# creare-com/pydem

Hardware: AMD Instinct MI355X
Metric: Mcells/s (slope+aspect+UCA+TWI end-to-end) per tile; % HBM roofline (higher is better)
Workload: dtype f64

## Files before the change

### pydem_amd/csrc/pits.hip

```cpp
#include "internal.h"
#include <hipcub/hipcub.hpp>
#include <math.h>
#include <stdlib.h>
#include <algorithm>
#include <vector>

namespace {

__device__ __forceinline__ double np_pairwise_leaf(const double *a, int n)
{
    if (n < 8) {
        double res = 0.;
        for (int i = 0; i < n; i++) res += a[i];
        return res;
    }
    double r0 = a[0], r1 = a[1], r2 = a[2], r3 = a[3], r4 = a[4], r5 = a[5], r6 = a[6], r7 = a[7];
    int i;
    for (i = 8; i < n - (n % 8); i += 8) {
        r0 += a[i]; r1 += a[i + 1]; r2 += a[i + 2]; r3 += a[i + 3];
        r4 += a[i + 4]; r5 += a[i + 5]; r6 += a[i + 6]; r7 += a[i + 7];
    }
    double res = ((r0 + r1) + (r2 + r3)) + ((r4 + r5) + (r6 + r7));
    for (; i < n; i++) res += a[i];
    return res;
// ... 1167 lines not shown
}

__global__ void k_pit_gather(const uint64_t *__restrict__ keys, const int32_t *__restrict__ idx, const double *__restrict__ w,
                             int32_t ne, int swap, int32_t *a, int32_t *b, double *wo, int32_t *dup, int kb)
{
    for (int32_t e = blockIdx.x * blockDim.x + threadIdx.x; e < ne; e += gridDim.x * blockDim.x) {
        const uint64_t k = keys[e];
        if (dup && e > 0 && keys[e - 1] == k) atomicAdd(dup, 1);
        const int32_t hi = (int32_t)(k >> kb), lo = (int32_t)(k & ((1ull << kb) - 1ull));
        a[e] = swap ? lo : hi;
        b[e] = swap ? hi : lo;
        wo[e] = w[idx[e]];
    }
}

template <typename T>
int dev_realloc(pydem_tile *t, T **p, size_t count)
{
    if (*p) { plane_give(t->device, *p); *p = nullptr; }
    return tile_alloc(t, p, count);
}

}

int stage_pits(pydem_tile *t, const pydem_options *opt)
{
    const int n = (int)t->n, m = (int)t->m;
    if (opt->drain_pits_max_iter > 300) {
        pydem_set_error("drain_pits_max_iter > 300 is not supported by the device window (got %d)", opt->drain_pits_max_iter);
        return -2;
    }
    HIP_TRY(hipEventRecord(t->ev[4], t->stream));
    PYDEM_TRY(tile_alloc(t, &t->flat0, (size_t)t->NN));
    PYDEM_TRY(tile_alloc(t, &t->flatlist, (size_t)t->NN));
    PYDEM_TRY(tile_alloc(t, &t->labels, (size_t)t->NN));
    PYDEM_TRY(tile_alloc(t, &t->queue[0], (size_t)t->NN));
    int32_t *cnt = t->counters + 40;
    HIP_TRY(hipMemsetAsync(cnt, 0, 16 * sizeof(int32_t), t->stream));
    const int big = (int)(cdiv(t->NN, 256) < 8192 ? cdiv(t->NN, 256) : 8192);
    hipLaunchKernelGGL(k_pitmask, dim3(big), dim3(256), 0, t->stream, t->flats, t->elev, t->NN, t->flat0);
    hipLaunchKernelGGL(k_compact_mask, dim3((unsigned)(cdiv(t->NN, 4096) < 4096 ? cdiv(t->NN, 4096) : 4096)), dim3(256), 0,
                       t->stream, t->flat0, t->NN, t->flatlist, cnt);
    HIP_TRY(hipMemcpyAsync(t->h_counters, cnt, sizeof(int32_t), hipMemcpyDeviceToHost, t->stream));
    HIP_TRY(hipStreamSynchronize(t->stream));
    const int32_t npits = t->h_counters[0];
    t->tm.n_pit_edges = 0; t->tm.n_pits_undrained = 0;
    t->tm.n_pits = npits; t->tm.n_pits_row = 0; t->tm.n_pits_wave = 0; t->tm.n_pits_big = 0;
    t->pits.n_edges = 0;
    if (npits == 0) { t->tm.pits_ms = 0; return 0; }

    int64_t cap = (int64_t)npits * 2 + 16384 * 4 * OUT_CHUNK + 1024;
    for (int attempt = 0;; attempt++) {
        if (t->pits.raw_cap < cap) {
            PYDEM_TRY(dev_realloc(t, &t->pits.raw_src, (size_t)cap));
            PYDEM_TRY(dev_realloc(t, &t->pits.raw_dst, (size_t)cap));
            PYDEM_TRY(dev_realloc(t, &t->pits.raw_w, (size_t)cap));
            t->pits.raw_cap = cap;
        }
        HIP_TRY(hipMemsetAsync(cnt + 1, 0, 8 * sizeof(int32_t), t->stream));
        PitParams P;
        P.dbg = nullptr; P.prof = nullptr;
        const char *dbg_env = getenv("PYDEM_PITS_DEBUG");
        if (dbg_env && atoi(dbg_env) == 3) { HIP_TRY(hipMalloc(&P.prof, 128)); HIP_TRY(hipMemsetAsync(P.prof, 0, 128, t->stream)); }
        if (dbg_env && atoi(dbg_env) >= 2) HIP_TRY(hipMalloc(&P.dbg, (size_t)npits * 16));
        HIP_TRY(hipMemsetAsync(t->pits.raw_src, 0xFF, (size_t)t->pits.raw_cap * 4, t->stream));
        P.elev = t->elev; P.pitmask = t->flat0; P.dX = t->dX; P.dY = t->dY; P.mag = t->mag; P.flats = t->flats;
        P.n = n; P.m = m; P.max_iter = opt->drain_pits_max_iter; P.max_dist = opt->drain_pits_max_dist;
        P.min_border = opt->drain_pits_min_border; P.max_dist_XY = opt->drain_pits_max_dist_XY;
        P.elev_f32 = t->elev_f32 ? 1 : 0;
        P.out_src = t->pits.raw_src; P.out_dst = t->pits.raw_dst; P.out_w = t->pits.raw_w;
        P.out_count = cnt + 1; P.out_cap = (int32_t)(t->pits.raw_cap < INT32_MAX ? t->pits.raw_cap : INT32_MAX);
        P.overflow_list = t->labels; P.overflow_count = cnt + 3;
        P.lane_overflow = t->queue[0];
        {
            static int handover = -1;
            if (handover < 0) { const char *e = getenv("PYDEM_PITS_HANDOVER"); handover = e ? atoi(e) : 1; }
            P.lane_state = nullptr;
            if (handover && (int64_t)npits * 12 <= t->NN) { PYDEM_TRY(tile_alloc(t, &t->queue[1], (size_t)t->NN)); P.lane_state = (uint32_t *)t->queue[1]; }
        }
        HIP_TRY(hipMemsetAsync(cnt + 10, 0, sizeof(int32_t), t->stream));
        P.work_next = cnt + 10;
        const int gl_cap = 3072 * 128 / LN_T;
        const int gl = (int)(cdiv(npits, LN_T) < gl_cap ? cdiv(npits, LN_T) : gl_cap);
        hipLaunchKernelGGL(k_pits_lane, dim3(gl), dim3(LN_T), 0, t->stream, P, t->flatlist, cnt);
        HIP_TRY(hipMemcpyAsync(t->h_counters, cnt, 8 * sizeof(int32_t), hipMemcpyDeviceToHost, t->stream));
        HIP_TRY(hipStreamSynchronize(t->stream));
        const int32_t n_lane_over = t->h_counters[5];
        if (P.prof) {
            unsigned long long h[8];
            HIP_TRY(hipMemcpy(h, P.prof, 64, hipMemcpyDeviceToHost));
            fprintf(stderr, "pits/lane: %llu loop trips over all wavefronts, %.1f busy lanes per trip; cycles: refill %llu, growth %llu, drain selection %llu, output %llu\n",
                    h[4], h[4] ? (double)h[3] / (double)h[4] : 0.0, h[0], h[5], h[1], h[2]);
        }
        int32_t n_row_over = -1, n_wave_over = 0, n_over = 0;
        P.wave_index = nullptr; P.row_overflow = nullptr; P.row_overflow_count = nullptr; P.row_rec = nullptr; P.rw_target = PYDEM_RW_TARGET;
        const char *row_env = getenv("PYDEM_PITS_ROW");
        const int row_mode = row_env ? atoi(row_env) : 1;
        const bool use_row = row_mode == 2 || (row_mode == 1 && n_lane_over >= 4 * 256 * PYDEM_WV_OCC);
        if (use_row && n_lane_over > 0 && 8 * (int64_t)n_lane_over + 64 <= t->NN) {
            HIP_TRY(hipMemsetAsync(cnt + 9, 0, 4 * sizeof(int32_t), t->stream));
            P.row_overflow = t->labels; P.row_overflow_count = cnt + 12;
            P.row_rec = (int2 *)(t->labels + (((size_t)t->NN / 2) & ~(size_t)63));
            const char *tgt_env = getenv("PYDEM_RW_TARGET");
            P.rw_target = tgt_env && atoi(tgt_env) > 0 ? atoi(tgt_env) : PYDEM_RW_TARGET;
            constexpr int per = RW_NT / 16, gr_cap = 256 * (RW_OCC * 256 / RW_NT);
            const int gr = (int)(cdiv(n_lane_over, per) < gr_cap ? cdiv(n_lane_over, per) : gr_cap);
            hipLaunchKernelGGL((k_pits_row<RW_CAP, RW_OCC, RW_NT>), dim3(gr), dim3(RW_NT), 0, t->stream, P, t->queue[0], cnt + 5);
            hipLaunchKernelGGL(k_pits_row_finish, dim3((unsigned)(cdiv(n_lane_over, 256) < 2048 ? cdiv(n_lane_over, 256) : 2048)), dim3(256), 0,
                               t->stream, P, t->queue[0], cnt + 5, P.row_rec);
            if (P.prof) {
                unsigned long long h[16];
                HIP_TRY(hipMemcpy(h, P.prof, 128, hipMemcpyDeviceToHost));
                fprintf(stderr, "pits/row: %llu loop trips over all wavefronts, %.2f busy / %.2f growing rows per trip, %llu refills; cycles: refill %llu, rounds %llu, drain selection %llu, output %llu\n",
                        h[12], h[12] ? (double)h[13] / (double)h[12] : 0.0, h[12] ? (double)h[14] / (double)h[12] : 0.0, h[15], h[8], h[9], h[10], h[11]);
            }
            P.wave_index = t->labels;
            P.overflow_list = t->labels + (((size_t)n_lane_over + 63) & ~(size_t)63);
            HIP_TRY(hipMemsetAsync(cnt + 10, 0, sizeof(int32_t), t->stream));
            const int gw = (int)(cdiv(n_lane_over, 4) < 256 * 4 ? cdiv(n_lane_over, 4) : 256 * 4);
            hipLaunchKernelGGL((k_pits_wave<512, 4>), dim3(gw), dim3(256), 0, t->stream, P, t->queue[0], cnt + 12);
            const int32_t *big_in = P.overflow_list;
            P.overflow_list = t->queue[0]; P.overflow_count = cnt + 9;
            P.wave_index = nullptr;
            hipLaunchKernelGGL(k_pits_wave_big, dim3(256), dim3(64), 0, t->stream, P, big_in, cnt + 3);
            HIP_TRY(hipMemcpyAsync(t->h_counters, cnt, 16 * sizeof(int32_t), hipMemcpyDeviceToHost, t->stream));
            HIP_TRY(hipStreamSynchronize(t->stream));
            n_row_over = t->h_counters[12]; n_wave_over = t->h_counters[3]; n_over = t->h_counters[9];
        } else {
            if (n_lane_over > 0) {
                const int gw = (int)(cdiv(n_lane_over, 4) < 256 * PYDEM_WV_OCC ? cdiv(n_lane_over, 4) : 256 * PYDEM_WV_OCC);
                HIP_TRY(hipMemsetAsync(cnt + 10, 0, sizeof(int32_t), t->stream));
                hipLaunchKernelGGL((k_pits_wave<PYDEM_WV_CAP, PYDEM_WV_OCC>), dim3(gw), dim3(256), 0, t->stream, P, t->queue[0], cnt + 5);
                HIP_TRY(hipMemcpyAsync(t->h_counters, cnt, 8 * sizeof(int32_t), hipMemcpyDeviceToHost, t->stream));
                HIP_TRY(hipStreamSynchronize(t->stream));
            }
            n_wave_over = t->h_counters[3];
            if (n_wave_over > 0) {
                HIP_TRY(hipMemsetAsync(cnt + 9, 0, sizeof(int32_t), t->stream));
                P.overflow_list = t->queue[0]; P.overflow_count = cnt + 9;
                hipLaunchKernelGGL(k_pits_wave_big, dim3(n_wave_over < 4096 ? n_wave_over : 4096), dim3(64), 0, t->stream, P, t->labels, cnt + 3);
                HIP_TRY(hipMemcpyAsync(t->h_counters, cnt, 16 * sizeof(int32_t), hipMemcpyDeviceToHost, t->stream));
                HIP_TRY(hipStreamSynchronize(t->stream));
                n_over = t->h_counters[9];
            }
        }
        if (P.prof) { (void)hipFree(P.prof); P.prof = nullptr; }
        t->tm.n_pits_row = n_row_over >= 0 ? n_lane_over : 0;
        t->tm.n_pits_wave = n_row_over >= 0 ? n_row_over : n_lane_over;
        t->tm.n_pits_big = n_wave_over;
        if (dbg_env) fprintf(stderr, "pits: %d candidates, %d left the 16x16 lane window, %d left the 64x64 row pass (-1: not run), %d left the 128x128 wavefront pass, %d left the 256x256 / 2048-cell pass, %d edge slots, %d undrained\n", npits, n_lane_over, n_row_over, n_wave_over, n_over, t->h_counters[1], t->h_counters[2]);
        if (P.dbg) {
            const int nrec = t->h_counters[7];
            std::vector<int32_t> rec((size_t)nrec * 4);
            HIP_TRY(hipMemcpy(rec.data(), P.dbg, rec.size() * 4, hipMemcpyDeviceToHost));
            (void)hipFree(P.dbg); P.dbg = nullptr;
            std::vector<int> rounds, border; int reason[4] = {0, 0, 0, 0}; long long tot_rounds = 0;
            for (int i = 0; i < nrec; i++) {
                rounds.push_back(rec[4 * i]); border.push_back(rec[4 * i + 1]); reason[rec[4 * i + 2] & 3]++; tot_rounds += rec[4 * i];
            }
            {
                const int edges[7] = {16, 32, 64, 128, 200, 299, 1 << 30};
                long long cr[7] = {0}, cn[7] = {0}, cd[7] = {0}, cu[7] = {0}, co[7] = {0};
                for (int i = 0; i < nrec; i++) {
                    int b = 0; while (rec[4 * i] > edges[b]) b++;
                    cr[b] += rec[4 * i]; cn[b]++;
                    if (rec[4 * i + 2] & 3) co[b]++; else if (rec[4 * i + 3] >= 0) cd[b]++; else cu[b]++;
// ... 115 lines not shown
```

### pydem_amd/csrc/uca.hip

```cpp
#include "uca_graph.h"
#include <algorithm>
#include <vector>
#include <math.h>
#include <stdlib.h>
#include <string.h>

#define PI_D 3.141592653589793

namespace {

__global__ __launch_bounds__(256) void k_section_proportion(const double *__restrict__ dir,
                                                            const uint8_t *__restrict__ flats,
                                                            const double *__restrict__ sec_theta, int64_t NN, int n, int m,
                                                            const double *__restrict__ elev,
                                                            int8_t *__restrict__ section, double *__restrict__ prop,
                                                            uint32_t *__restrict__ cinfo)
{
    (void)NN;
    for (int i = blockIdx.y; i < n; i += gridDim.y)
    for (int j = blockIdx.x * blockDim.x + threadIdx.x; j < m; j += gridDim.x * blockDim.x) {
        const int64_t c = (int64_t)i * m + j;
        const double theta = sec_theta[i];
        const double d = dir[c];
        int sec0 = (int)(int8_t)(int)floor(d / PI_D * 2.0);
        const double quadrant = d - PI_D / 2.0 * (double)sec0;
        const int mod2 = sec0 & 1;
        int sec = sec0 * 2 + ((quadrant > theta) && mod2 == 0) + ((quadrant > (PI_D / 2 - theta)) && mod2 == 1);
        sec = (int)(int8_t)sec;
        const bool I1 = sec == 0 || sec == 1 || sec == 4 || sec == 5;
        const double cth = PI_D / 2 - theta;
        const double t1 = I1 ? theta : cth, t2 = I1 ? cth : theta;
        const bool lo = quadrant <= t1, hi = quadrant > t1;
        const double num = lo ? quadrant : quadrant - t1, den = lo ? t1 : t2;
        double p = (lo || hi) ? num / den : NAN;
        if (flats[c]) { sec = -1; p = NAN; }
        if (sec == 8) sec = 0;
        const int a = (sec & 1) ? -1 : 1;
        const double pf = (1 + a) / 2.0 - (double)a * p;
        prop[c] = pf;
        section[c] = (int8_t)sec;
        uint32_t gf = 0;
        if (sec >= 0 && sec <= 7) {
            const double z = elev[c];
            const int i1 = i + fe1r(sec), j1 = j + fe1c(sec), i2 = i + fe2r(sec), j2 = j + fe2c(sec);
            if (i1 >= 0 && i1 < n && j1 >= 0 && j1 < m && keep_edge(pf, elev[(int64_t)i1 * m + j1], z)) gf |= CI_OUT1;
            if (i2 >= 0 && i2 < n && j2 >= 0 && j2 < m && keep_edge(1 - pf, elev[(int64_t)i2 * m + j2], z)) gf |= CI_OUT2;
        }
        cinfo[c] = gf | ((uint32_t)(sec & 7) << CI_SEC_SHIFT);
    }
}

__global__ __launch_bounds__(256) void k_graph_inmask(const double *__restrict__ prop, const double *__restrict__ elev,
                                                      int n, int m, uint32_t *__restrict__ cinfo, uint8_t *__restrict__ todo0,
                                                      uint8_t *__restrict__ todo_work, double *__restrict__ corner_sums)
{
    for (int i = blockIdx.y; i < n; i += gridDim.y)
    for (int j = blockIdx.x * blockDim.x + threadIdx.x; j < m; j += gridDim.x * blockDim.x) {
        const int64_t c = (int64_t)i * m + j;
        const uint32_t cw = cinfo[c] & (CI_OUT1 | CI_OUT2 | (7u << CI_SEC_SHIFT));
        uint32_t im = 0;
#pragma unroll
        for (int d = 0; d < 8; d++) {
            const int ui = i + NB_DI[d], uj = j + NB_DJ[d];
            if (ui < 0 || ui >= n || uj < 0 || uj >= m) continue;
            const uint32_t wu = cinfo[(int64_t)ui * m + uj];
            const int su = (int)((wu >> CI_SEC_SHIFT) & 7u);
            const bool cardinal = (NB_DI[d] == 0) || (NB_DJ[d] == 0);
            if ((su == NB_S0[d] || su == NB_S1[d]) && (wu & (cardinal ? CI_OUT1 : CI_OUT2))) im |= 1u << d;
        }
        cinfo[c] = im | cw | ((im ? CI_LEVEL_INF : 0u) << CI_LEVEL_SHIFT);
        const bool top = i == 0, bot = i == n - 1, left = j == 0, right = j == m - 1;
        if (top || bot || left || right) {
            const double TOL = 1e-2;
            const double p = prop[c], z = elev[c];
            double outsum = 0.0;
            if (cw & CI_OUT1) outsum += p;
            if (cw & CI_OUT2) outsum += 1 - p;
            const int s = (cw & (CI_OUT1 | CI_OUT2)) ? ci_section(cw) : -1;
            bool td = false;
            const bool has_out = outsum > TOL;
            if (left) td = has_out && (s == 6 || s == 7 || s == 0 || s == 1);
            if (right) td = has_out && (s == 2 || s == 3 || s == 4 || s == 5);
            if (top) td = has_out && (s == 4 || s == 5 || s == 6 || s == 7);
            if (bot) td = has_out && (s == 0 || s == 1 || s == 2 || s == 3);
            if ((top || bot) && (left || right)) {
                double insum = 0.0;
                for (int d = 0; d < 8; d++)
                    if (im & (1u << d)) {
                        const int64_t u = (int64_t)(i + NB_DI[d]) * m + (j + NB_DJ[d]);
                        const bool cardinal = (NB_DI[d] == 0) || (NB_DJ[d] == 0);
                        insum += cardinal ? prop[u] : 1 - prop[u];
                    }
                const int q = (top ? 0 : 2) + (left ? 0 : 1);
                corner_sums[q * 3 + 0] = outsum;
                corner_sums[q * 3 + 1] = insum;
                corner_sums[q * 3 + 2] = td ? 1.0 : 0.0;
            }
            if (isnan(z)) td = false;
            todo0[c] = td;
            todo_work[c] = td;
        }
    }
}

__global__ void k_graph_add_pits(const int32_t *__restrict__ src, const int32_t *__restrict__ dst,
                                 const double *__restrict__ w, int64_t ne, int n, int m,
                                 uint32_t *cinfo, double *corner_sums)
{
    for (int64_t e = (int64_t)blockIdx.x * blockDim.x + threadIdx.x; e < ne; e += (int64_t)gridDim.x * blockDim.x) {
        const int32_t s = src[e], d = dst[e];
        atomicOr(&cinfo[s], CI_PIT_OUT);
        atomicOr(&cinfo[d], CI_PIT_IN | (CI_LEVEL_INF << CI_LEVEL_SHIFT));
        const int corners[4] = {0, m - 1, (n - 1) * m, (n - 1) * m + m - 1};
        for (int q = 0; q < 4; q++) {
            if (s == corners[q]) atomicAdd(&corner_sums[q * 3 + 0], w[e]);
            if (d == corners[q]) atomicAdd(&corner_sums[q * 3 + 1], w[e]);
        }
    }
}

__global__ void k_corner_todo(const double *__restrict__ corner_sums, const double *__restrict__ elev, int n, int m,
                              uint8_t *todo0, uint8_t *todo_work)
{
    const int q = threadIdx.x;
    if (q >= 4) return;
    const int64_t corners[4] = {0, m - 1, (int64_t)(n - 1) * m, (int64_t)(n - 1) * m + m - 1};
    const int64_t c = corners[q];
    bool td = corner_sums[q * 3 + 2] != 0.0;
    td = td || (corner_sums[q * 3 + 0] > 1e-2) || (corner_sums[q * 3 + 1] < 1e-2);
    if (isnan(elev[c])) td = false;
    todo0[c] = td;
    todo_work[c] = td;
}

constexpr int STAGE_CAP = 4096;
constexpr int STAGE_FLUSH = STAGE_CAP - 512;


struct Stage {
    QE buf[STAGE_CAP];
    int32_t cnt;
    int32_t base;
};

__device__ __forceinline__ void stage_push(Stage &S, bool pred, int32_t cell, uint32_t cw)
{
    const unsigned long long bal = __ballot(pred);
    if (bal == 0ull) return;
    const int lane = (int)__lane_id();
    const int leader = __ffsll((long long)bal) - 1;
    int32_t base = 0;
    if (lane == leader) base = atomicAdd(&S.cnt, (int32_t)__popcll(bal));
    base = __shfl(base, leader);
    if (pred) { QE q; q.c = cell; q.cw = cw; S.buf[base + __popcll(bal & ((1ull << lane) - 1ull))] = q; }
}

__device__ __forceinline__ void stage_flush(const SweepArgs &A, Stage &S, QE *__restrict__ qn, int32_t *cn, bool force)
{
    __syncthreads();
    const int32_t c = S.cnt;
    if (c > 0 && (force || c > STAGE_FLUSH)) {
        if (threadIdx.x == 0) S.base = atomicAdd(cn, c);
        __syncthreads();
        const int32_t b = S.base;
        if ((int64_t)b + c <= A.qcap) { for (int32_t k = threadIdx.x; k < c; k += blockDim.x) qn[b + k] = S.buf[k]; }
        else if (threadIdx.x == 0) atomicAdd(A.err, 1);
        __syncthreads();
        if (threadIdx.x == 0) S.cnt = 0;
    }
    __syncthreads();
}

__device__ __forceinline__ int2 pit_stash(const SweepArgs &A, int32_t c) { return reinterpret_cast<const int2 *>(A.area)[c]; }

__global__ void k_pit_stash(const int32_t *__restrict__ pin_dst, const int32_t *__restrict__ pit_src, int64_t ne, double *area)
{
    int32_t *slots = reinterpret_cast<int32_t *>(area);
    for (int64_t e = (int64_t)blockIdx.x * blockDim.x + threadIdx.x; e < ne; e += (int64_t)gridDim.x * blockDim.x) {
        if (e == 0 || pin_dst[e - 1] != pin_dst[e]) slots[2 * (int64_t)pin_dst[e]] = (int32_t)e;
        if (e == 0 || pit_src[e - 1] != pit_src[e]) slots[2 * (int64_t)pit_src[e] + 1] = (int32_t)e;
    }
}

__device__ __forceinline__ void load_upstream_words(const SweepArgs &A, int32_t t, int ti, int tj, uint32_t w[8])
// ... 1401 lines not shown
template <bool WT = false>
__global__ __launch_bounds__(256) void k_reseed_gather(SweepArgs A, const ReseedCell *__restrict__ U, int32_t nU, const double *__restrict__ elev,
                                                       ReseedHost *__restrict__ out)
{
    for (int32_t k = blockIdx.x * blockDim.x + threadIdx.x; k < nU; k += gridDim.x * blockDim.x) {
        ReseedHost h;
        h.c = U[k].c; h.cw = A.cinfo[h.c] & CI_STATIC_MASK; h.pin_first = U[k].pin_first; h.pout_first = U[k].pout_first;
        double a; bool td;
        gather_finished<WT>(A, h.c, h.cw, h.pin_first, a, td);
        h.area = a; h.td = td; h.pad = 0; h.elev = elev[h.c]; h.prop = (h.cw & (CI_OUT1 | CI_OUT2)) ? A.prop[h.c] : 0.0;
        out[k] = h;
    }
}
struct ReseedBack { int32_t c; int32_t flags; double area; };
__global__ __launch_bounds__(256) void k_reseed_scatter(SweepArgs A, const ReseedBack *__restrict__ B, int32_t nU, uint32_t pass)
{
    for (int32_t k = blockIdx.x * blockDim.x + threadIdx.x; k < nU; k += gridDim.x * blockDim.x) {
        const int32_t c = B[k].c;
        A.area[c] = B[k].area;
        if (B[k].flags & 2) A.todo_work[c] = 1;
        if (B[k].flags & 1) A.cinfo[c] = ci_with_level(A.cinfo[c], pass);
    }
}

__device__ __forceinline__ bool finalize_cell(double *__restrict__ uca, const double *__restrict__ elev, int64_t c, uint32_t f, uint32_t td,
                                              int apply_limit, double limit)
{
    if (f) uca[c] = NAN;
    bool dn = !td;
    if (td && isnan(elev[c])) dn = true;
    if (apply_limit && !f && uca[c] > limit) dn = true;
    return dn;
}

__global__ __launch_bounds__(256) void k_uca_finalize(double *__restrict__ uca, const uint8_t *__restrict__ flats,
                                                      const uint8_t *__restrict__ todo_work, const double *__restrict__ elev,
                                                      uint8_t *__restrict__ edge_done, int64_t NN, int apply_limit, double limit)
{
    const int64_t nvec = NN >> 4, stride = (int64_t)gridDim.x * blockDim.x, t0 = (int64_t)blockIdx.x * blockDim.x + threadIdx.x;
    for (int64_t v = t0; v < nvec; v += stride) {
        const uint4 f4 = reinterpret_cast<const uint4 *>(flats)[v], t4 = reinterpret_cast<const uint4 *>(todo_work)[v];
        const uint32_t fw[4] = {f4.x, f4.y, f4.z, f4.w}, tw[4] = {t4.x, t4.y, t4.z, t4.w};
        uint32_t dw[4];
#pragma unroll
        for (int q = 0; q < 4; q++) {
            uint32_t d = 0;
#pragma unroll
            for (int b = 0; b < 4; b++)
                d |= (finalize_cell(uca, elev, v * 16 + q * 4 + b, (fw[q] >> (8 * b)) & 0xFFu, (tw[q] >> (8 * b)) & 0xFFu, apply_limit, limit) ? 1u : 0u) << (8 * b);
            dw[q] = d;
        }
        reinterpret_cast<uint4 *>(edge_done)[v] = make_uint4(dw[0], dw[1], dw[2], dw[3]);
    }
    for (int64_t c = (nvec << 4) + t0; c < NN; c += stride)
        edge_done[c] = finalize_cell(uca, elev, c, flats[c], todo_work[c], apply_limit, limit);
}

__global__ __launch_bounds__(256) void k_twi(const double *__restrict__ uca, const double *__restrict__ mag,
                                             double *__restrict__ twi, int64_t NN, double min_slope, int lim_uca,
                                             double uca_cap, int lim_twi, double twi_cap)
{
    for (int64_t c = (int64_t)blockIdx.x * blockDim.x + threadIdx.x; c < NN; c += (int64_t)gridDim.x * blockDim.x) {
        double t = uca[c];
        if (lim_uca && t > uca_cap) t = uca_cap;
        t = log(t / (mag[c] + min_slope));
        if (lim_twi && t > twi_cap) t = twi_cap;
        twi[c] = t;
    }
}

}

int stage_section_graph(pydem_tile *t, const pydem_options *opt)
{
    const int n = (int)t->n, m = (int)t->m;
    t->graph_opt = *opt;
    t->edge_clean = false;
    t->einc_ready = false;
    PYDEM_TRY(tile_alloc(t, &t->todo_work, (size_t)t->NN));
    PYDEM_TRY(tile_alloc(t, &t->cinfo, (size_t)t->NN));
    const dim3 grid2((unsigned)(cdiv(m, 256) < 64 ? cdiv(m, 256) : 64), (unsigned)(n < 16384 ? n : 16384));
    t->tm.n_pit_edges = 0; t->tm.n_pits_undrained = 0; t->tm.pits_ms = 0;
    t->pits.n_edges = 0; t->pits.n_raw = 0;
    double *corner_sums = (double *)(t->counters + CS_WORK);
    HIP_TRY(hipEventRecord(t->ev_fork, t->stream));
    HIP_TRY(hipStreamWaitEvent(t->stream2, t->ev_fork, 0));
    HIP_TRY(hipMemcpyAsync(t->todo_work, t->flats, (size_t)t->NN, hipMemcpyDeviceToDevice, t->stream2));
    HIP_TRY(hipEventRecord(t->ev_snap, t->stream2));
    HIP_TRY(hipStreamWaitEvent(t->stream, t->ev_snap, 0));
    hipLaunchKernelGGL(k_section_proportion, grid2, dim3(256), 0, t->stream2, t->dir, (const uint8_t *)t->todo_work, t->sec_theta,
                       t->NN, n, m, t->elev, t->section, t->prop, t->cinfo);
    HIP_TRY(hipMemsetAsync(t->counters + CS_WORK, 0, CS_WORK_WORDS * sizeof(int32_t), t->stream2));
    HIP_TRY(hipMemsetAsync(t->edge_todo, 0, (size_t)t->NN, t->stream2));
    HIP_TRY(hipMemsetAsync(t->todo_work, 0, (size_t)t->NN, t->stream2));
    hipLaunchKernelGGL(k_graph_inmask, grid2, dim3(256), 0, t->stream2, t->prop, t->elev, n, m,
                       t->cinfo, t->edge_todo, t->todo_work, corner_sums);
    HIP_TRY(hipEventRecord(t->ev_join, t->stream2));
    static int graph_serial = -1;
    if (graph_serial < 0) { const char *e = getenv("PYDEM_GRAPH_SERIAL"); graph_serial = e ? atoi(e) : 0; }
    if (graph_serial) HIP_TRY(hipStreamWaitEvent(t->stream, t->ev_join, 0));
    HIP_TRY(hipEventRecord(t->ev[0], t->stream));
    if (opt->drain_pits) PYDEM_TRY(stage_pits(t, opt));
    HIP_TRY(hipEventRecord(t->ev[2], t->stream));
    HIP_TRY(hipStreamWaitEvent(t->stream, t->ev_join, 0));
    if (t->pits.n_edges > 0) {
        hipLaunchKernelGGL(k_graph_add_pits, dim3(grid_for(t->pits.n_edges, 1024)), dim3(256), 0, t->stream, t->pits.src,
                           t->pits.dst, t->pits.w, t->pits.n_edges, n, m, t->cinfo, corner_sums);
    }
    hipLaunchKernelGGL(k_corner_todo, dim3(1), dim3(64), 0, t->stream, corner_sums, t->elev, n, m, t->edge_todo, t->todo_work);
    HIP_TRY(hipEventRecord(t->ev[3], t->stream));
    HIP_TRY(hipGetLastError());
    HIP_TRY(hipEventSynchronize(t->ev[3]));
    float a = 0, b = 0;
    HIP_TRY(hipEventElapsedTime(&a, t->ev[0], t->ev[2]));
    HIP_TRY(hipEventElapsedTime(&b, t->ev[2], t->ev[3]));
    (void)a;
    t->tm.graph_ms = b;
    return 0;
}


static int64_t reseed_replay_host(std::vector<ReseedHost> &H, std::vector<uint8_t> &done, int n, int m, int maxcount, bool tile_has_nan,
                                  const std::vector<int32_t> &pit_src, const std::vector<int32_t> &pit_dst, const std::vector<double> &pit_w,
                                  const std::vector<int32_t> &pin_dst, const std::vector<int32_t> &pin_src)
{
    const int32_t nU = (int32_t)H.size();
    const int64_t n_pit = (int64_t)pit_src.size();
    static const int DI[8] = {-1, -1, -1, 0, 0, 1, 1, 1}, DJ[8] = {-1, 0, 1, -1, 1, -1, 0, 1};
    auto find = [&](int32_t c) -> int32_t {
        int32_t lo = 0, hi = nU - 1;
        while (lo <= hi) { const int32_t mid = (lo + hi) >> 1; if (H[(size_t)mid].c == c) return mid; if (H[(size_t)mid].c < c) lo = mid + 1; else hi = mid - 1; }
        return -1;
    };
    auto on_edge = [&](int32_t c) { const int i = c / m, j = c - i * m; return i == 0 || i == n - 1 || j == 0 || j == m - 1; };
    auto is_done = [&](int32_t c) -> bool { const int32_t k = find(c); return k < 0 || done[(size_t)k]; };
    done.assign((size_t)nU, 0);
    std::vector<uint8_t> in_cur((size_t)nU, 0);
    std::vector<int32_t> cur, prev;
    int64_t n_done = 0, done_prev = -1;
    for (int count = 2; n_done < nU && count < maxcount && n_done != done_prev; count++) {
        done_prev = n_done;
        double mx = 0.0;
        for (int32_t k = 0; k < nU; k++) if (!done[(size_t)k] && H[(size_t)k].elev > mx) mx = H[(size_t)k].elev;
        if (tile_has_nan) mx = NAN;
        cur.clear();
        for (int32_t k = 0; k < nU; k++) {
            const double v = done[(size_t)k] ? 0.0 : H[(size_t)k].elev;
            if ((v - mx) / mx > -0.01) cur.push_back(k);
        }
        for (int64_t guard = 0; guard < 8 * (int64_t)nU + 64; guard++) {
            for (int32_t k : cur) { if (!done[(size_t)k]) n_done++; done[(size_t)k] = 1; }
            prev.swap(cur); cur.clear();
            for (int32_t k : prev) {
                const ReseedHost &S = H[(size_t)k];
                const int32_t i = S.c;
                int32_t tg[2]; double fc[2]; int nt = 0;
                if (S.cw & (CI_OUT1 | CI_OUT2)) {
                    const int sct = (int)((S.cw >> CI_SEC_SHIFT) & 7u);
                    if (S.cw & CI_OUT1) { tg[nt] = i + fe1r(sct) * m + fe1c(sct); fc[nt] = S.prop; nt++; }
                    if (S.cw & CI_OUT2) { tg[nt] = i + fe2r(sct) * m + fe2c(sct); fc[nt] = 1 - S.prop; nt++; }
                    if (nt == 2 && tg[1] < tg[0]) { std::swap(tg[0], tg[1]); std::swap(fc[0], fc[1]); }
                }
                int64_t e = (S.cw & CI_PIT_OUT) ? S.pout_first : 0;
                for (int q = 0;; q++) {
                    int32_t row; double factor;
                    if (S.cw & CI_PIT_OUT) { if (!(e < n_pit && pit_src[(size_t)e] == i)) break; row = pit_dst[(size_t)e]; factor = pit_w[(size_t)e]; e++; }
                    else { if (q >= nt) break; row = tg[q]; factor = fc[q]; }
                    const int32_t kr = find(row);
                    if (kr < 0) continue;
                    if (done[(size_t)kr] && on_edge(row)) continue;
                    H[(size_t)kr].area += S.area * factor;
                    if (S.td) H[(size_t)kr].td = 1;
                    bool wait = false;
                    const uint32_t cwr = H[(size_t)kr].cw;
                    for (int d = 0; d < 8 && !wait; d++)
                        if ((cwr & (1u << d)) && !is_done(row + DI[d] * m + DJ[d])) wait = true;
                    if (!wait && (cwr & CI_PIT_IN))
                        for (int64_t e2 = H[(size_t)kr].pin_first; e2 < n_pit && pin_dst[(size_t)e2] == row; e2++)
                            if (!is_done(pin_src[(size_t)e2])) { wait = true; break; }
// ... 444 lines not shown
```

Before: 5649.

## Add fused strip-band graph build kernel behind env flag, defer pits wait on snapshot

Factors the per-cell section/proportion, out-edge and in-mask logic into helpers. It adds a fused k_graph_build kernel that streams rows through a wavefront-wide register window with lane shuffles, computing section, prop and cinfo in one pass instead of two. A small border kernel then handles the todo_work and corner sums. The fused path is only enabled when PYDEM_GRAPH_FUSED is set. The main stream's wait on the flats snapshot event moves from before the section kernel launch to just before the pits lane kernel, so pits setup can overlap the snapshot copy.

```diff
diff --git a/pydem_amd/csrc/pits.hip b/pydem_amd/csrc/pits.hip
--- a/pydem_amd/csrc/pits.hip
+++ b/pydem_amd/csrc/pits.hip
@@ -1273,6 +1273,7 @@
         P.work_next = cnt + 10;
         const int gl_cap = 3072 * 128 / LN_T;
         const int gl = (int)(cdiv(npits, LN_T) < gl_cap ? cdiv(npits, LN_T) : gl_cap);
+        HIP_TRY(hipStreamWaitEvent(t->stream, t->ev_snap, 0));
         hipLaunchKernelGGL(k_pits_lane, dim3(gl), dim3(LN_T), 0, t->stream, P, t->flatlist, cnt);
         HIP_TRY(hipMemcpyAsync(t->h_counters, cnt, 8 * sizeof(int32_t), hipMemcpyDeviceToHost, t->stream));
         HIP_TRY(hipStreamSynchronize(t->stream));
diff --git a/pydem_amd/csrc/uca.hip b/pydem_amd/csrc/uca.hip
--- a/pydem_amd/csrc/uca.hip
+++ b/pydem_amd/csrc/uca.hip
@@ -9,6 +9,81 @@
 
 namespace {
 
+
+__device__ __forceinline__ void cell_section_prop(double d, double theta, bool flat, int &sec_out, double &pf_out)
+{
+    int sec0 = (int)(int8_t)(int)floor(d / PI_D * 2.0);
+    const double quadrant = d - PI_D / 2.0 * (double)sec0;
+    const int mod2 = sec0 & 1;
+    int sec = sec0 * 2 + ((quadrant > theta) && mod2 == 0) + ((quadrant > (PI_D / 2 - theta)) && mod2 == 1);
+    sec = (int)(int8_t)sec;
+    const bool I1 = sec == 0 || sec == 1 || sec == 4 || sec == 5;
+    const double cth = PI_D / 2 - theta;
+    const double t1 = I1 ? theta : cth, t2 = I1 ? cth : theta;
+    const bool lo = quadrant <= t1, hi = quadrant > t1;
+    const double num = lo ? quadrant : quadrant - t1, den = lo ? t1 : t2;
+    double p = (lo || hi) ? num / den : NAN;
+    if (flat) { sec = -1; p = NAN; }
+    if (sec == 8) sec = 0;
+    const int a = (sec & 1) ? -1 : 1;
+    pf_out = (1 + a) / 2.0 - (double)a * p;
+    sec_out = sec;
+}
+
+__device__ __forceinline__ uint32_t cell_out_word(int sec, double pf, double z, double z1, double z2)
+{
+    uint32_t gf = 0;
+    if (sec >= 0 && sec <= 7) {
+        if (keep_edge(pf, z1, z)) gf |= CI_OUT1;
+        if (keep_edge(1 - pf, z2, z)) gf |= CI_OUT2;
+    }
+    return gf | ((uint32_t)(sec & 7) << CI_SEC_SHIFT);
+}
+
+__device__ __forceinline__ uint32_t cell_in_bit(uint32_t wu, int d)
+{
+    const int su = (int)((wu >> CI_SEC_SHIFT) & 7u);
+    const bool cardinal = (NB_DI[d] == 0) || (NB_DJ[d] == 0);
+    const uint32_t points_here = (uint32_t)(su == NB_S0[d]) | (uint32_t)(su == NB_S1[d]);
+    return (points_here & ((wu & (cardinal ? CI_OUT1 : CI_OUT2)) != 0u ? 1u : 0u)) << d;
+}
+
+__device__ __forceinline__ uint32_t cell_graph_word(uint32_t im, uint32_t cw)
+{
+    return im | cw | ((im ? CI_LEVEL_INF : 0u) << CI_LEVEL_SHIFT);
+}
+
+__device__ __forceinline__ bool cell_inlet_todo(uint32_t cw, double p, bool top, bool bot, bool left, bool right, double &outsum)
+{
+    const double TOL = 1e-2;
+    outsum = 0.0;
+    if (cw & CI_OUT1) outsum += p;
+    if (cw & CI_OUT2) outsum += 1 - p;
+    const int s = (cw & (CI_OUT1 | CI_OUT2)) ? ci_section(cw) : -1;
+    bool td = false;
+    const bool has_out = outsum > TOL;
+    if (left) td = has_out && (s == 6 || s == 7 || s == 0 || s == 1);
+    if (right) td = has_out && (s == 2 || s == 3 || s == 4 || s == 5);
+    if (top) td = has_out && (s == 4 || s == 5 || s == 6 || s == 7);
+    if (bot) td = has_out && (s == 0 || s == 1 || s == 2 || s == 3);
+    return td;
+}
+
+__device__ __forceinline__ void corner_sums_of(const double *__restrict__ prop, int i, int j, int m, uint32_t im, double outsum, bool td,
+                                               int q, double *__restrict__ corner_sums)
+{
+    double insum = 0.0;
+    for (int d = 0; d < 8; d++)
+        if (im & (1u << d)) {
+            const int64_t u = (int64_t)(i + NB_DI[d]) * m + (j + NB_DJ[d]);
+            const bool cardinal = (NB_DI[d] == 0) || (NB_DJ[d] == 0);
+            insum += cardinal ? prop[u] : 1 - prop[u];
+        }
+    corner_sums[q * 3 + 0] = outsum;
+    corner_sums[q * 3 + 1] = insum;
+    corner_sums[q * 3 + 2] = td ? 1.0 : 0.0;
+}
+
 __global__ __launch_bounds__(256) void k_section_proportion(const double *__restrict__ dir,
                                                             const uint8_t *__restrict__ flats,
                                                             const double *__restrict__ sec_theta, int64_t NN, int n, int m,
@@ -20,33 +95,17 @@
     for (int i = blockIdx.y; i < n; i += gridDim.y)
     for (int j = blockIdx.x * blockDim.x + threadIdx.x; j < m; j += gridDim.x * blockDim.x) {
         const int64_t c = (int64_t)i * m + j;
-        const double theta = sec_theta[i];
-        const double d = dir[c];
-        int sec0 = (int)(int8_t)(int)floor(d / PI_D * 2.0);
-        const double quadrant = d - PI_D / 2.0 * (double)sec0;
-        const int mod2 = sec0 & 1;
-        int sec = sec0 * 2 + ((quadrant > theta) && mod2 == 0) + ((quadrant > (PI_D / 2 - theta)) && mod2 == 1);
-        sec = (int)(int8_t)sec;
-        const bool I1 = sec == 0 || sec == 1 || sec == 4 || sec == 5;
-        const double cth = PI_D / 2 - theta;
-        const double t1 = I1 ? theta : cth, t2 = I1 ? cth : theta;
-        const bool lo = quadrant <= t1, hi = quadrant > t1;
-        const double num = lo ? quadrant : quadrant - t1, den = lo ? t1 : t2;
-        double p = (lo || hi) ? num / den : NAN;
-        if (flats[c]) { sec = -1; p = NAN; }
-        if (sec == 8) sec = 0;
-        const int a = (sec & 1) ? -1 : 1;
-        const double pf = (1 + a) / 2.0 - (double)a * p;
+        int sec; double pf;
+        cell_section_prop(dir[c], sec_theta[i], flats[c] != 0, sec, pf);
         prop[c] = pf;
         section[c] = (int8_t)sec;
-        uint32_t gf = 0;
+        double z1 = NAN, z2 = NAN;
         if (sec >= 0 && sec <= 7) {
-            const double z = elev[c];
             const int i1 = i + fe1r(sec), j1 = j + fe1c(sec), i2 = i + fe2r(sec), j2 = j + fe2c(sec);
-            if (i1 >= 0 && i1 < n && j1 >= 0 && j1 < m && keep_edge(pf, elev[(int64_t)i1 * m + j1], z)) gf |= CI_OUT1;
-            if (i2 >= 0 && i2 < n && j2 >= 0 && j2 < m && keep_edge(1 - pf, elev[(int64_t)i2 * m + j2], z)) gf |= CI_OUT2;
-        }
-        cinfo[c] = gf | ((uint32_t)(sec & 7) << CI_SEC_SHIFT);
+            if (i1 >= 0 && i1 < n && j1 >= 0 && j1 < m) z1 = elev[(int64_t)i1 * m + j1];
+            if (i2 >= 0 && i2 < n && j2 >= 0 && j2 < m) z2 = elev[(int64_t)i2 * m + j2];
+        }
+        cinfo[c] = cell_out_word(sec, pf, elev[c], z1, z2);
     }
 }
 
@@ -63,43 +122,164 @@
         for (int d = 0; d < 8; d++) {
             const int ui = i + NB_DI[d], uj = j + NB_DJ[d];
             if (ui < 0 || ui >= n || uj < 0 || uj >= m) continue;
-            const uint32_t wu = cinfo[(int64_t)ui * m + uj];
-            const int su = (int)((wu >> CI_SEC_SHIFT) & 7u);
-            const bool cardinal = (NB_DI[d] == 0) || (NB_DJ[d] == 0);
-            if ((su == NB_S0[d] || su == NB_S1[d]) && (wu & (cardinal ? CI_OUT1 : CI_OUT2))) im |= 1u << d;
-        }
-        cinfo[c] = im | cw | ((im ? CI_LEVEL_INF : 0u) << CI_LEVEL_SHIFT);
+            im |= cell_in_bit(cinfo[(int64_t)ui * m + uj], d);
+        }
+        cinfo[c] = cell_graph_word(im, cw);
         const bool top = i == 0, bot = i == n - 1, left = j == 0, right = j == m - 1;
         if (top || bot || left || right) {
-            const double TOL = 1e-2;
-            const double p = prop[c], z = elev[c];
-            double outsum = 0.0;
-            if (cw & CI_OUT1) outsum += p;
-            if (cw & CI_OUT2) outsum += 1 - p;
-            const int s = (cw & (CI_OUT1 | CI_OUT2)) ? ci_section(cw) : -1;
-            bool td = false;
-            const bool has_out = outsum > TOL;
-            if (left) td = has_out && (s == 6 || s == 7 || s == 0 || s == 1);
-            if (right) td = has_out && (s == 2 || s == 3 || s == 4 || s == 5);
-            if (top) td = has_out && (s == 4 || s == 5 || s == 6 || s == 7);
-            if (bot) td = has_out && (s == 0 || s == 1 || s == 2 || s == 3);
-            if ((top || bot) && (left || right)) {
-                double insum = 0.0;
-                for (int d = 0; d < 8; d++)
-                    if (im & (1u << d)) {
-                        const int64_t u = (int64_t)(i + NB_DI[d]) * m + (j + NB_DJ[d]);
-                        const bool cardinal = (NB_DI[d] == 0) || (NB_DJ[d] == 0);
-                        insum += cardinal ? prop[u] : 1 - prop[u];
-                    }
-                const int q = (top ? 0 : 2) + (left ? 0 : 1);
-                corner_sums[q * 3 + 0] = outsum;
-                corner_sums[q * 3 + 1] = insum;
-                corner_sums[q * 3 + 2] = td ? 1.0 : 0.0;
-            }
-            if (isnan(z)) td = false;
+            double outsum;
+            bool td = cell_inlet_todo(cw, prop[c], top, bot, left, right, outsum);
+            if ((top || bot) && (left || right)) corner_sums_of(prop, i, j, m, im, outsum, td, (top ? 0 : 2) + (left ? 0 : 1), corner_sums);
+            if (isnan(elev[c])) td = false;
             todo0[c] = td;
             todo_work[c] = td;
         }
+    }
+}
+
+constexpr int GB_COLS = 2;
+constexpr int GB_WINDOW = 64 * GB_COLS;
+constexpr int GB_STRIP = GB_WINDOW - 4;
+constexpr int GB_BAND = 128;
+
+template <typename T> __device__ __forceinline__ T lane_prev(T v, int lane) { return __shfl(v, (lane + 63) & 63, 64); }
+template <typename T> __device__ __forceinline__ T lane_next(T v, int lane) { return __shfl(v, (lane + 1) & 63, 64); }
+
+template <typename T> __device__ __forceinline__ void window_neighbours(const T (&v)[GB_COLS], int lane, T outside, T (&l)[GB_COLS], T (&r)[GB_COLS])
+{
+    T p[GB_COLS], q[GB_COLS];
+#pragma unroll
+    for (int k = 0; k < GB_COLS; k++) { p[k] = lane_prev(v[k], lane); q[k] = lane_next(v[k], lane); }
+#pragma unroll
+    for (int k = 0; k < GB_COLS; k++) {
+        l[k] = lane != 0 ? p[k] : (k > 0 ? p[k > 0 ? k - 1 : 0] : outside);
+        r[k] = lane != 63 ? q[k] : (k < GB_COLS - 1 ? q[k < GB_COLS - 1 ? k + 1 : k] : outside);
+    }
+}
+
+__device__ __forceinline__ double pick9(int di, int dj, double ul, double uc, double ur, double cl, double cc, double cr, double dl, double dc,
+                                        double dr)
+{
+    const double l = di < 0 ? ul : (di > 0 ? dl : cl), c = di < 0 ? uc : (di > 0 ? dc : cc), r = di < 0 ? ur : (di > 0 ? dr : cr);
+    return dj < 0 ? l : (dj > 0 ? r : c);
+}
+
+__global__ __launch_bounds__(64) void k_graph_build(const double *__restrict__ dir, const uint8_t *__restrict__ flats,
+                                                    const double *__restrict__ sec_theta, const double *__restrict__ elev, int n, int m,
+                                                    int n_strips, int8_t *__restrict__ section, double *__restrict__ prop, uint32_t *__restrict__ cinfo,
+                                                    uint8_t *__restrict__ todo0)
+{
+    const int lane = (int)threadIdx.x;
+    const int band = (int)(blockIdx.x / (unsigned)n_strips), strip = (int)(blockIdx.x - (unsigned)band * (unsigned)n_strips);
+    const int b0 = band * GB_BAND, b1 = b0 + GB_BAND < n ? b0 + GB_BAND : n;
+    int col[GB_COLS]; bool inside[GB_COLS], own[GB_COLS];
+#pragma unroll
+    for (int k = 0; k < GB_COLS; k++) {
+        const int wi = k * 64 + lane;
+        col[k] = strip * GB_STRIP - 2 + wi;
+        inside[k] = col[k] >= 0 && col[k] < m;
+        own[k] = inside[k] && wi >= 2 && wi < GB_WINDOW - 2;
+    }
+    double zu[GB_COLS], zul[GB_COLS], zur[GB_COLS], zc[GB_COLS], zcl[GB_COLS], zcr[GB_COLS], zd[GB_COLS], zdl[GB_COLS], zdr[GB_COLS];
+    uint32_t wu[GB_COLS], wul[GB_COLS], wur[GB_COLS], wc[GB_COLS], wcl[GB_COLS], wcr[GB_COLS], wd[GB_COLS], wdl[GB_COLS], wdr[GB_COLS];
+    double pc[GB_COLS];
+#pragma unroll
+    for (int k = 0; k < GB_COLS; k++) {
+        zc[k] = zcl[k] = zcr[k] = zd[k] = zdl[k] = zdr[k] = NAN;
+        wc[k] = wcl[k] = wcr[k] = wd[k] = wdl[k] = wdr[k] = 0u;
+        pc[k] = NAN;
+    }
+    double nz[GB_COLS], nd[GB_COLS]; uint8_t nf[GB_COLS];
+    auto load_step = [&](int s) {
+#pragma unroll
+        for (int k = 0; k < GB_COLS; k++) {
+            nz[k] = (inside[k] && s >= 0 && s < n) ? elev[(int64_t)s * m + col[k]] : NAN;
+            const bool rw = inside[k] && s - 1 >= 0 && s - 1 < n && s - 1 >= b0 - 1;
+            nd[k] = rw ? dir[(int64_t)(s - 1) * m + col[k]] : NAN;
+            nf[k] = rw ? flats[(int64_t)(s - 1) * m + col[k]] : (uint8_t)0;
+        }
+    };
+    load_step(b0 - 2);
+    for (int s = b0 - 2; s <= b1 + 1; s++) {
+        double dcur[GB_COLS]; uint8_t fcur[GB_COLS];
+#pragma unroll
+        for (int k = 0; k < GB_COLS; k++) {
+            zu[k] = zc[k]; zul[k] = zcl[k]; zur[k] = zcr[k]; zc[k] = zd[k]; zcl[k] = zdl[k]; zcr[k] = zdr[k];
+            wu[k] = wc[k]; wul[k] = wcl[k]; wur[k] = wcr[k]; wc[k] = wd[k]; wcl[k] = wdl[k]; wcr[k] = wdr[k];
+            zd[k] = nz[k]; dcur[k] = nd[k]; fcur[k] = nf[k];
+        }
+        if (s < b1 + 1) load_step(s + 1);
+        window_neighbours(zd, lane, (double)NAN, zdl, zdr);
+        const int i = s - 1;
+        const bool row_in = i >= 0 && i < n;
+        const double theta = sec_theta[row_in ? i : 0];
+        double pd[GB_COLS];
+#pragma unroll
+        for (int k = 0; k < GB_COLS; k++) { wd[k] = 0u; pd[k] = NAN; }
+        if (i >= b0 - 1)
+#pragma unroll
+        for (int k = 0; k < GB_COLS; k++) {
+            int sec; double pf;
+            cell_section_prop(dcur[k], theta, fcur[k] != 0, sec, pf);
+            const int sk = sec & 7;
+            const double z1 = pick9(fe1r(sk), fe1c(sk), zul[k], zu[k], zur[k], zcl[k], zc[k], zcr[k], zdl[k], zd[k], zdr[k]);
+            const double z2 = pick9(fe2r(sk), fe2c(sk), zul[k], zu[k], zur[k], zcl[k], zc[k], zcr[k], zdl[k], zd[k], zdr[k]);
+            wd[k] = (row_in && inside[k]) ? cell_out_word(sec, pf, zc[k], z1, z2) : 0u;
+            pd[k] = pf;
+            if (own[k] && i >= b0 && i < b1) {
+                const int64_t c = (int64_t)i * m + col[k];
+                prop[c] = pf;
+                section[c] = (int8_t)sec;
+            }
+        }
+        window_neighbours(wd, lane, 0u, wdl, wdr);
+        const int r = s - 2;
+        if (r >= b0 && r < b1) {
+#pragma unroll
+            for (int k = 0; k < GB_COLS; k++) {
+                if (!own[k]) continue;
+                const uint32_t nbw[8] = {wul[k], wu[k], wur[k], wcl[k], wcr[k], wdl[k], wd[k], wdr[k]};
+                uint32_t im = 0;
+#pragma unroll
+                for (int d = 0; d < 8; d++) im |= cell_in_bit(nbw[d], d);
+                const int64_t c = (int64_t)r * m + col[k];
+                cinfo[c] = cell_graph_word(im, wc[k]);
+                const bool top = r == 0, bot = r == n - 1, left = col[k] == 0, right = col[k] == m - 1;
+                if (top || bot || left || right) {
+                    double outsum;
+                    const bool td = cell_inlet_todo(wc[k], pc[k], top, bot, left, right, outsum);
+                    todo0[c] = td && !isnan(zu[k]);
+                }
+            }
+        }
+#pragma unroll
+        for (int k = 0; k < GB_COLS; k++) pc[k] = pd[k];
+    }
+}
+
+__global__ __launch_bounds__(256) void k_graph_border(const double *__restrict__ prop, const uint32_t *__restrict__ cinfo, int n, int m,
+                                                      const uint8_t *__restrict__ todo0, uint8_t *__restrict__ todo_work,
+                                                      double *__restrict__ corner_sums)
+{
+    const int64_t per = 2 * ((int64_t)n + m);
+    for (int64_t p = (int64_t)blockIdx.x * blockDim.x + threadIdx.x; p < per; p += (int64_t)gridDim.x * blockDim.x) {
+        int64_t c;
+        if (p < m) c = p;
+        else if (p < 2 * (int64_t)m) c = (int64_t)(n - 1) * m + (p - m);
+        else if (p < 2 * (int64_t)m + n) c = (p - 2 * (int64_t)m) * m;
+        else c = (p - 2 * (int64_t)m - n) * m + (m - 1);
+        todo_work[c] = todo0[c];
+    }
+    if (blockIdx.x == 0 && threadIdx.x < 4) {
+        const int q = (int)threadIdx.x;
+        const bool top = q < 2, left = (q & 1) == 0;
+        const int i = top ? 0 : n - 1, j = left ? 0 : m - 1;
+        const int64_t c = (int64_t)i * m + j;
+        const uint32_t w = cinfo[c];
+        double outsum;
+        const bool ctop = i == 0, cleft = j == 0;
+        const bool td = cell_inlet_todo(w & (CI_OUT1 | CI_OUT2 | (7u << CI_SEC_SHIFT)), prop[c], ctop, i == n - 1, cleft, j == m - 1, outsum);
+        if (q == (ctop ? 0 : 2) + (cleft ? 0 : 1)) corner_sums_of(prop, i, j, m, w & 0xFFu, outsum, td, q, corner_sums);
     }
 }
 
@@ -1667,19 +1847,29 @@
     const dim3 grid2((unsigned)(cdiv(m, 256) < 64 ? cdiv(m, 256) : 64), (unsigned)(n < 16384 ? n : 16384));
     t->tm.n_pit_edges = 0; t->tm.n_pits_undrained = 0; t->tm.pits_ms = 0;
     t->pits.n_edges = 0; t->pits.n_raw = 0;
+    const char *fused_env = getenv("PYDEM_GRAPH_FUSED");
+    const bool fused = fused_env ? atoi(fused_env) != 0 : false;
     double *corner_sums = (double *)(t->counters + CS_WORK);
     HIP_TRY(hipEventRecord(t->ev_fork, t->stream));
     HIP_TRY(hipStreamWaitEvent(t->stream2, t->ev_fork, 0));
     HIP_TRY(hipMemcpyAsync(t->todo_work, t->flats, (size_t)t->NN, hipMemcpyDeviceToDevice, t->stream2));
     HIP_TRY(hipEventRecord(t->ev_snap, t->stream2));
-    HIP_TRY(hipStreamWaitEvent(t->stream, t->ev_snap, 0));
-    hipLaunchKernelGGL(k_section_proportion, grid2, dim3(256), 0, t->stream2, t->dir, (const uint8_t *)t->todo_work, t->sec_theta,
-                       t->NN, n, m, t->elev, t->section, t->prop, t->cinfo);
     HIP_TRY(hipMemsetAsync(t->counters + CS_WORK, 0, CS_WORK_WORDS * sizeof(int32_t), t->stream2));
     HIP_TRY(hipMemsetAsync(t->edge_todo, 0, (size_t)t->NN, t->stream2));
-    HIP_TRY(hipMemsetAsync(t->todo_work, 0, (size_t)t->NN, t->stream2));
-    hipLaunchKernelGGL(k_graph_inmask, grid2, dim3(256), 0, t->stream2, t->prop, t->elev, n, m,
-                       t->cinfo, t->edge_todo, t->todo_work, corner_sums);
+    if (fused) {
+        const int64_t n_strips = cdiv(m, GB_STRIP), n_bands = cdiv(n, GB_BAND);
+        hipLaunchKernelGGL(k_graph_build, dim3((unsigned)(n_strips * n_bands)), dim3(64), 0, t->stream2, t->dir, (const uint8_t *)t->todo_work,
+                           t->sec_theta, t->elev, n, m, (int)n_strips, t->section, t->prop, t->cinfo, t->edge_todo);
+        HIP_TRY(hipMemsetAsync(t->todo_work, 0, (size_t)t->NN, t->stream2));
+        hipLaunchKernelGGL(k_graph_border, dim3(grid_for(2 * ((int64_t)n + m), 64)), dim3(256), 0, t->stream2, t->prop, t->cinfo, n, m,
+                           t->edge_todo, t->todo_work, corner_sums);
+    } else {
+        hipLaunchKernelGGL(k_section_proportion, grid2, dim3(256), 0, t->stream2, t->dir, (const uint8_t *)t->todo_work, t->sec_theta,
+                           t->NN, n, m, t->elev, t->section, t->prop, t->cinfo);
+        HIP_TRY(hipMemsetAsync(t->todo_work, 0, (size_t)t->NN, t->stream2));
+        hipLaunchKernelGGL(k_graph_inmask, grid2, dim3(256), 0, t->stream2, t->prop, t->elev, n, m,
+                           t->cinfo, t->edge_todo, t->todo_work, corner_sums);
+    }
     HIP_TRY(hipEventRecord(t->ev_join, t->stream2));
     static int graph_serial = -1;
     if (graph_serial < 0) { const char *e = getenv("PYDEM_GRAPH_SERIAL"); graph_serial = e ? atoi(e) : 0; }
```

Result: slower. 5523 (-2.2%).
